# facebookresearch/unbiased-teacher-v2

Measured on AMD Instinct MI355X. Metric: images/sec/node (labeled+unlabeled) UTv2 step, R50-FPN 1333x800, higher is better.
Workload: dtype f16

## Files before the change

include/utv2.h:

```cpp
#ifndef UTV2_H
#define UTV2_H
#include <stdint.h>
#ifdef __cplusplus
extern "C" {
#endif

typedef struct ihipStream_t* utv2_stream_t;

int utv2_conv2d_nhwc_fwd(const float* x, const float* w, float* y, const float* scale, const float* bias,
                         const float* residual, int N, int H, int W, int C, int K, int KH, int KW, int stride, int pad,
                         int in_dil, int OH, int OW, int relu, int accumulate, int Kred, utv2_stream_t stream);
int utv2_conv2d_stem_fwd(const float* x, const float* w, void* y, int y_dtype, const float* scale, const float* bias, int N,
                         int H, int W, int K, int KH, int KW, int stride, int pad, int OH, int OW, int relu, int Kred,
                         utv2_stream_t stream);
int utv2_conv2d_wgrad_splits(int N, int OH, int OW, int K, int Kred);
int64_t utv2_conv2d_wgrad_workspace_floats(int N, int OH, int OW, int K, int Kred);
int utv2_conv2d_nhwc_wgrad(const float* x, const float* dy, float* dw, float* ws, int N, int H, int W, int C, int K,
                           int KH, int KW, int stride, int pad, int OH, int OW, int accumulate, utv2_stream_t stream);
int utv2_colsum(const float* g, float* db, float* ws, int M, int C, int accumulate, utv2_stream_t stream);
int utv2_weight_flip_transpose(const float* w, float* wt, int K, int KH, int KW, int C, utv2_stream_t stream);

int utv2_conv2d_ml_fwd(const float* x, const float* w, float* y, const float* scale, const float* bias,
                       const float* residual, int nlev, const int* H_host, const int* W_host, int N, int C, int K, int KH,
                       int KW, int pad, int relu, int accumulate, utv2_stream_t stream);
// ... 9 lines not shown
int utv2_conv2d_nhwc_fwd_bf16_bits(const void* x, int x_dtype, const void* w16, void* y, int y_dtype, const float* scale,
                                   const float* bias, const void* residual, const void* mask, const void* post_mask, int N, int H, int W,
                                   int C, int K, int KH, int KW, int stride, int pad, int in_dil, int OH, int OW, int relu, int accumulate,
                                   const int* rowinfo, void* relu_bits, const void* mask_bits, const void* post_mask_bits,
                                   utv2_stream_t stream);
int utv2_conv2d_ml_fwd_bf16_g(const void* x, int x_dtype, int x_pitch, const void* w16, void* y, int y_dtype, int y_pitch,
                              const float* scale, const float* bias, const void* residual, int nlev, const int* H_host,
                              const int* W_host, int N, int C, int K, int KH, int KW, int pad, int relu, int accumulate, int groups,
                              float* gn_part, const int* rowinfo, utv2_stream_t stream);
int utv2_conv2d_ml_fwd_bf16_gnb(const void* x, int x_pitch, const void* w16, void* y, int nlev, const int* H_host, const int* W_host, int N,
                                int C, int K, int KH, int KW, int pad, int groups, const int* rowinfo, const void* mask_bits,
                                const void* gnb_x, float* gnb_part, utv2_stream_t stream);
int utv2_conv2d_wgrad_bf16_splits(int M, int K, int Kred);
int64_t utv2_conv2d_wgrad_bf16_workspace_floats(int M, int K, int Kred);
int utv2_conv2d_wgrad_bf16_g(const void* x, int x_dtype, int x_pitch, const void* dy, int dy_dtype, int dy_pitch, float* dw, float* db,
                             float* ws, const int* rowinfo, const float* rowscale, int M, int C, int K, int KH, int KW, int accumulate,
                             int groups, utv2_stream_t stream);
int utv2_conv2d_wgrad_bf16_d(const void* x, int x_dtype, int x_pitch, const void* dy, int dy_dtype, int dy_pitch, float* dw, float* db,
                             float* ws, const int* rowinfo, const float* rowscale, int M, int C, int K, int KH, int KW, int accumulate,
                             int groups, void* pending, utv2_stream_t stream);
int64_t utv2_wgrad_fold_table_bytes(void);
int utv2_wgrad_fold_pending(const void* pending);
int utv2_wgrad_fold_flush(void* pending, utv2_stream_t stream);
int utv2_conv2d_stem_fwd_bf16(const void* xpad16, const void* w16s, void* y, int y_dtype, const float* scale,
                              const float* bias, int N, int H, int W, int K, int OH, int OW, int relu, utv2_stream_t stream);
int utv2_rowinfo_nhwc(int* out, int N, int H, int W, int OH, int OW, int stride, int pad, int KH, int KW, int64_t start,
                      utv2_stream_t stream);
int utv2_f32_to_bf16(const float* src, void* dst16, int64_t n, utv2_stream_t stream);
int utv2_weight_flip_transpose_bf16(const float* w, void* wt16, const float* scale, int K, int KH, int KW, int C,
                                    utv2_stream_t stream);
int utv2_pad_cols_bf16(const void* src, int src_dtype, void* dst16, int64_t rows, int c, int cpad, utv2_stream_t stream);
int utv2_weight_flip_transpose_bf16_batched(const float* arena, const float* scales, void* bank, const void* table, int nlayers,
                                            utv2_stream_t stream);

int utv2_ema_axpby(float* teacher, const float* student, int64_t n, double keep_rate, utv2_stream_t stream);
int utv2_sgd_momentum(float* param, float* grad, float* mom_buf, int64_t n, float lr, float momentum, float weight_decay,
                      float grad_scale, int zero_grad, utv2_stream_t stream);
int utv2_amp_found_inf(const float* grad, int64_t n, float* state, utv2_stream_t stream);
int utv2_sgd_momentum_amp(float* param, const float* grad, float* mom_buf, int64_t n, float lr, float momentum, float weight_decay,
                          float grad_scale, const float* state, utv2_stream_t stream);
int utv2_amp_update_scale(float* state, float growth_factor, float backoff_factor, int growth_interval, utv2_stream_t stream);
int utv2_ema_axpby_m16(float* teacher, const float* student, void* mirror16, int64_t n, double keep_rate, utv2_stream_t stream);
int utv2_sgd_momentum_m16(float* param, float* grad, float* mom_buf, void* mirror16, int64_t n, float lr, float momentum, float weight_decay,
                          float grad_scale, int zero_grad, utv2_stream_t stream);
int utv2_sgd_momentum_amp_m16(float* param, const float* grad, float* mom_buf, void* mirror16, int64_t n, float lr, float momentum,
                              float weight_decay, float grad_scale, const float* state, utv2_stream_t stream);
// ... 242 lines not shown
```

unbiased-teacher-v2_amd/csrc/conv_bf16.hip:

```cpp
#include <mutex>
#include <stdlib.h>
#include "common.h"
#include <type_traits>

__device__ uint4 g_zero64[4] = {{0, 0, 0, 0}, {0, 0, 0, 0}, {0, 0, 0, 0}, {0, 0, 0, 0}};

#define CONV_MAX_LEVELS 8
struct LevelTab {
  int n;
  int start[CONV_MAX_LEVELS + 1];
  int H[CONV_MAX_LEVELS], W[CONV_MAX_LEVELS];
};

struct ConvArgs16 {
  LevelTab lt;
  const void* x;
  const h16_t* w;
  void* y;
  const float* scale;
  const float* bias;
  const void* residual;
  const void* mask;
  const void* post_mask;
  int N, H, W, C, OH, OW, K, KH, KW, stride, pad, in_dil, relu, Kred, M, accumulate;
// ... 1464 lines not shown

int utv2_weight_flip_transpose_bf16_batched(const float* arena, const float* scales, void* bank, const void* table, int nlayers,
                                            hipStream_t stream) {
  if (!arena || !bank || !table || nlayers < 1) return UTV2_EARG;
  static_assert(sizeof(FlipDesc) == 48, "table record layout is part of the ABI");
  hipLaunchKernelGGL(weight_flip_transpose_bf16_batched_kernel, dim3(512, nlayers), dim3(256), 0, stream, arena, scales, (h16_t*)bank,
                     (const FlipDesc*)table);
  return utv2_launch_status();
}

}

struct Wgrad16Args {
  const void* x;
  const void* dy;
  float* ws;
  const int2* rowinfo;
  float* bias_ws;
  int C, K, KH, KW, Kred, M, splits, chunks_per_split;
  int xs;
  int groups;
  int dys;
  int debug;
};

__device__ __forceinline__ bf16x4_t lds_read_tr16(const unsigned char* p) {
  typedef short s16x4 __attribute__((ext_vector_type(4)));
  const s16x4 v = __builtin_amdgcn_ds_read_tr16_b64_v4i16((__attribute__((address_space(3))) s16x4*)p);
  return __builtin_bit_cast(bf16x4_t, v);
}

template <typename TX, typename TDY>
__global__ __launch_bounds__(256) void conv_wgrad_bf16(Wgrad16Args p) {
  constexpr int BK = 32, LDR = 320;
  constexpr int OPB = BK * LDR;
  constexpr bool X16 = sizeof(TX) == 2, DY16 = sizeof(TDY) == 2;
  __shared__ __attribute__((aligned(16))) unsigned char smem[2 * 2 * OPB];
  const int tid = threadIdx.x, lane = tid & 63, wid = tid >> 6;
  const int wm = wid >> 1, wn = wid & 1;
  const int tilesN = (p.Kred + 127) / 128, tilesM = (p.K + 127) / 128;
  const int tiles = tilesM * tilesN;
  int split, bid;
  if ((p.splits & 7) == 0) {
    const int xcd = blockIdx.x & 7, idx = blockIdx.x >> 3;
    split = xcd + 8 * (idx / tiles);
    bid = idx % tiles;
  } else {
    split = blockIdx.x / tiles;
    bid = blockIdx.x - split * tiles;
  }
  const int mt = bid / tilesN, nt = bid - mt * tilesN;
  const int i0 = mt * 128, j0 = nt * 128;
  const int goff = p.groups > 1 ? (i0 / (p.K / p.groups)) * p.C : 0;

  const int cg = tid & 15, pl0 = tid >> 4;
  const int co8 = i0 + cg * 8;
  const bool aok = co8 < p.K;
  const int kk = j0 + cg * 8;
  const bool bok = kk < p.Kred;
  const int tap = bok ? kk / p.C : 0;
  const int ci = bok ? kk - tap * p.C : 0;
  const int dh = tap / p.KW, dw = tap - dh * p.KW;

  f32x16 acc[2][2];
#pragma unroll
  for (int i = 0; i < 2; ++i)
#pragma unroll
    for (int j = 0; j < 2; ++j)
#pragma unroll
      for (int e = 0; e < 16; ++e) acc[i][j][e] = 0.f;

  const int chunk_begin = split * p.chunks_per_split;
  const int total_chunks = (p.M + BK - 1) / BK;
  int chunk_end = chunk_begin + p.chunks_per_split;
  if (chunk_end > total_chunks) chunk_end = total_chunks;

  int2 ri[2];
  bf16x8_t ra[2], rb[2];
  float bsum[8];
#pragma unroll
  for (int e = 0; e < 8; ++e) bsum[e] = 0.f;
  const bool do_bias = p.bias_ws != nullptr && nt == 0;

  auto rload = [&](int chunk) {
#pragma unroll
    for (int r = 0; r < 2; ++r) {
      int m = chunk * BK + pl0 + 16 * r;
      m = m < p.M ? m : p.M - 1;
      ri[r] = p.rowinfo[m];
    }
  };
  auto load8 = [&](const void* base, size_t eoff, bool is16, bool ok) -> bf16x8_t {
    bf16x8_t v;
    if (is16) {
      const h16_t* src = ok ? (const h16_t*)base + eoff : (const h16_t*)g_zero64;
      v = *(const bf16x8_t*)src;
    } else {
      const float* src = ok ? (const float*)base + eoff : (const float*)g_zero64;
      const f32x4 v0 = *(const f32x4*)src, v1 = *(const f32x4*)(src + 4);
#pragma unroll
      for (int e = 0; e < 4; ++e) {
        v[e] = (h16_t)v0[e];
        v[4 + e] = (h16_t)v1[e];
      }
    }
    return v;
  };
  auto load_piece = [&](int chunk, int q) {
    const int r = q & 1;
    const int m = chunk * BK + pl0 + 16 * r;
    const bool mok = m < p.M;
    if (q < 2) {
      ra[r] = load8(p.dy, (size_t)m * p.dys + co8, DY16, mok && aok);
    } else {
      const int W = ri[r].y >> 16;
      const bool ok = mok && bok && ((ri[r].y >> tap) & 1);
      rb[r] = load8(p.x, (size_t)(ri[r].x + dh * W + dw) * p.xs + goff + ci, X16, ok);
    }
  };
  auto store_piece = [&](int buf, int q) {
    const int r = q & 1;
    unsigned char* dst = smem + buf * 2 * OPB + (q < 2 ? 0 : OPB) + (pl0 + 16 * r) * LDR + cg * 16;
    if (q < 2) {
      *(bf16x8_t*)dst = ra[r];
      if (do_bias) {
#pragma unroll
        for (int e = 0; e < 8; ++e) bsum[e] += (float)ra[r][e];
      }
    } else {
      *(bf16x8_t*)dst = rb[r];
    }
  };

  const int G = lane >> 4, t = lane & 15;
// ... 346 lines not shown
  __shared__ float red[256];
  const int c = blockIdx.x * 32 + (threadIdx.x & 31), part = threadIdx.x >> 5;
  float s[4] = {0.f, 0.f, 0.f, 0.f};
  if (c < K) {
    int b = part;
    for (; b + 24 < nb; b += 32) {
#pragma unroll
      for (int u = 0; u < 4; ++u) s[u] += partial[(size_t)(b + 8 * u) * K + c];
    }
    for (; b < nb; b += 8) s[0] += partial[(size_t)b * K + c];
  }
  red[threadIdx.x] = (s[0] + s[1]) + (s[2] + s[3]);
  __syncthreads();
  if (part == 0 && c < K) {
    float v = 0.f;
#pragma unroll
    for (int k = 0; k < 8; ++k) v += red[threadIdx.x + 32 * k];
    if (rowscale) v *= rowscale[c];
    db[c] = accumulate ? db[c] + v : v;
  }
}

__global__ __launch_bounds__(256) void reduce_slabs16_f32(const float* __restrict__ ws, float* __restrict__ dst, size_t n, int splits,
                                                          int accumulate, const float* __restrict__ rowscale, int rowlen) {
  const size_t n4 = n >> 2;
  size_t i = (size_t)blockIdx.x * blockDim.x + threadIdx.x;
  const size_t stride = (size_t)gridDim.x * blockDim.x;
  for (; i < n4; i += stride) {
    f32x4 s[4];
#pragma unroll
    for (int u = 0; u < 4; ++u) s[u] = f32x4{0.f, 0.f, 0.f, 0.f};
    int k = 0;
    for (; k + 4 <= splits; k += 4) {
#pragma unroll
      for (int u = 0; u < 4; ++u) s[u] += ((const f32x4*)(ws + (size_t)(k + u) * n))[i];
    }
    for (; k < splits; ++k) s[0] += ((const f32x4*)(ws + (size_t)k * n))[i];
    f32x4 t = (s[0] + s[1]) + (s[2] + s[3]);
    if (rowscale) {
      const float r = rowscale[(i * 4) / rowlen];
#pragma unroll
      for (int e = 0; e < 4; ++e) t[e] *= r;
    }
    if (accumulate) t += ((const f32x4*)dst)[i];
    ((f32x4*)dst)[i] = t;
  }
}

__global__ void reduce_slabs16_scalar_f32(const float* __restrict__ ws, float* __restrict__ dst, size_t n, int splits, int accumulate,
                                          const float* __restrict__ rowscale) {
  size_t i = (size_t)blockIdx.x * blockDim.x + threadIdx.x;
  if (i >= n) return;
  float s = 0.f;
  for (int k = 0; k < splits; ++k) s += ws[(size_t)k * n + i];
  if (rowscale) s *= rowscale[i];
  dst[i] = accumulate ? dst[i] + s : s;
}

#define SLAB_FOLD_MAX 24
struct SlabFold {
  const float* ws;
  float* dst;
  const float* rowscale;
  unsigned long long n;
  int splits, accumulate, rowlen, kind;
  int blk0, nblk;
};
struct SlabFoldTable {
  int count, total_blocks;
  SlabFold e[SLAB_FOLD_MAX];
};

__global__ __launch_bounds__(256) void reduce_slabs_table(SlabFoldTable t) {
  __shared__ float red[256];
  int ei = 0;
  for (int i = 1; i < t.count; ++i)
    if ((int)blockIdx.x >= t.e[i].blk0) ei = i;
  const SlabFold f = t.e[ei];
  const int lb = (int)blockIdx.x - f.blk0;
  if (f.kind == 0) {
    const size_t n4 = f.n >> 2;
    const size_t stride = (size_t)f.nblk * 256;
    for (size_t i = (size_t)lb * 256 + threadIdx.x; i < n4; i += stride) {
      f32x4 s[4];
#pragma unroll
      for (int u = 0; u < 4; ++u) s[u] = f32x4{0.f, 0.f, 0.f, 0.f};
      int k = 0;
      for (; k + 4 <= f.splits; k += 4) {
#pragma unroll
        for (int u = 0; u < 4; ++u) s[u] += ((const f32x4*)(f.ws + (size_t)(k + u) * f.n))[i];
      }
      for (; k < f.splits; ++k) s[0] += ((const f32x4*)(f.ws + (size_t)k * f.n))[i];
      f32x4 v = (s[0] + s[1]) + (s[2] + s[3]);
      if (f.rowscale) {
        const float r = f.rowscale[(i * 4) / f.rowlen];
#pragma unroll
        for (int e = 0; e < 4; ++e) v[e] *= r;
      }
      if (f.accumulate) v += ((const f32x4*)f.dst)[i];
      ((f32x4*)f.dst)[i] = v;
    }
// ... 8 lines not shown
    const int K = (int)f.n, nb = f.splits;
    const int c = lb * 32 + (threadIdx.x & 31), part = threadIdx.x >> 5;
    float s[4] = {0.f, 0.f, 0.f, 0.f};
    if (c < K) {
      int b = part;
      for (; b + 24 < nb; b += 32) {
#pragma unroll
        for (int u = 0; u < 4; ++u) s[u] += f.ws[(size_t)(b + 8 * u) * K + c];
      }
      for (; b < nb; b += 8) s[0] += f.ws[(size_t)b * K + c];
    }
    red[threadIdx.x] = (s[0] + s[1]) + (s[2] + s[3]);
    __syncthreads();
    if (part == 0 && c < K) {
      float v = 0.f;
#pragma unroll
      for (int k = 0; k < 8; ++k) v += red[threadIdx.x + 32 * k];
      if (f.rowscale) v *= f.rowscale[c];
      f.dst[c] = f.accumulate ? f.dst[c] + v : v;
    }
  }
}

static int slab_fold_add(SlabFoldTable* t, int kind, const float* ws, float* dst, const float* rowscale, size_t n, int splits, int accumulate,
                         int rowlen) {
  if (t->count < 0 || t->count >= SLAB_FOLD_MAX) return UTV2_EARG;
  for (int i = 0; i < t->count; ++i)
    if (t->e[i].dst == dst) return UTV2_EARG;
  SlabFold& f = t->e[t->count];
  f.kind = kind; f.ws = ws; f.dst = dst; f.rowscale = rowscale; f.n = n; f.splits = splits; f.accumulate = accumulate; f.rowlen = rowlen;
  int nb;
  if (kind == 0) { nb = cdiv((int64_t)n / 4, 256); if (nb > 2048) nb = 2048; }
  else if (kind == 1) nb = cdiv((int64_t)n, 256);
  else nb = cdiv((int64_t)n, 32);
  if (nb < 1) nb = 1;
  f.blk0 = t->count == 0 ? 0 : t->e[t->count - 1].blk0 + t->e[t->count - 1].nblk;
  f.nblk = nb;
  t->total_blocks = f.blk0 + nb;
  ++t->count;
  return UTV2_OK;
}

extern "C" {

static int wgrad16_small_splits(int M, int K, int Kred) {
  const int chunks = cdiv(M, 32);
  const int tiles = cdiv(K, 128) * cdiv(Kred, 128);
  const double flop = 2.0 * M * K * Kred;
  int splits = cdiv(flop > 512 * 2.0e8 ? 1024 : 512, tiles);
  const int max_by_chunks = chunks / 8 > 0 ? chunks / 8 : 1;
  if (splits > max_by_chunks) splits = max_by_chunks;
  if (splits < 1) splits = 1;
  if (splits > 256) splits = 256;
// ... 23 lines not shown
    return false;
  if (KH * KW == 1 && chunks < 16 * (256 / tiles)) return false;
  return true;
}

int utv2_conv2d_wgrad_bf16_splits(int M, int K, int Kred) { return wgrad16_small_splits(M, K, Kred); }

int utv2_colsum_partials(const float* partial, float* db, int nb, int K, int accumulate, hipStream_t stream) {
  if (!partial || !db || nb < 1 || K < 1) return UTV2_EARG;
  hipLaunchKernelGGL(colsum_final_f32, dim3(cdiv(K, 32)), dim3(256), 0, stream, partial, db, nb, K, accumulate, (const float*)nullptr);
  return utv2_launch_status();
}

int64_t utv2_conv2d_wgrad_bf16_workspace_floats(int M, int K, int Kred) {
  int64_t n = (int64_t)wgrad16_small_splits(M, K, Kred) * ((int64_t)K * Kred + K);
  if ((K & 255) == 0 && (Kred & 255) == 0) {
    const int64_t n8 = (int64_t)wgrad16_w8_splits(M, K, Kred) * K * Kred + (int64_t)WGRAD_W8_MAX_NB * K;
    if (n8 > n) n = n8;
  }
  return n;
}

static int wgrad16_tail(SlabFoldTable* pending, int kind, const float* src, float* dst, const float* rowscale, size_t n, int parts,
                        int accumulate, int rowlen, hipStream_t stream) {
  if (pending) return slab_fold_add(pending, kind, src, dst, rowscale, n, parts, accumulate, rowlen);
  if (kind == 0) {
    int rb = cdiv((int64_t)n / 4, 256);
    if (rb > 8192) rb = 8192;
    hipLaunchKernelGGL(reduce_slabs16_f32, dim3(rb), dim3(256), 0, stream, src, dst, n, parts, accumulate, rowscale, rowlen);
  } else if (kind == 1) {
    hipLaunchKernelGGL(reduce_slabs16_scalar_f32, dim3(cdiv((int64_t)n, 256)), dim3(256), 0, stream, src, dst, n, parts, accumulate, rowscale);
  } else {
    hipLaunchKernelGGL(colsum_final_f32, dim3(cdiv((int64_t)n, 32)), dim3(256), 0, stream, src, dst, parts, (int)n, accumulate, rowscale);
  }
  return UTV2_OK;
}

static int wgrad_bf16_impl(const void* x, int x_dtype, int x_pitch, const void* dy, int dy_dtype, int dy_pitch, float* dw, float* db,
                           float* ws, const int* rowinfo, const float* rowscale, int M, int C, int K, int KH, int KW, int accumulate,
                           int groups, hipStream_t stream, SlabFoldTable* pending) {
  if (!x || !dy || !dw || !ws || !rowinfo || (C & 7) || (K & 7) || M <= 0 || KH * KW > 16 || bad_dtype(x_dtype) ||
      bad_dtype(dy_dtype) || groups < 1 || K % groups || x_pitch < groups * C || (groups > 1 && (K / groups) % 128) ||
      (x_pitch != C && (x_pitch & (x_dtype == UTV2_BF16 ? 7 : 3))) || dy_pitch < K || (dy_pitch != K && (dy_pitch & (dy_dtype == UTV2_BF16 ? 7 : 3))))
    return UTV2_EARG;
  Wgrad16Args a;
  a.x = x; a.dy = dy; a.ws = ws; a.rowinfo = (const int2*)rowinfo;
  a.C = C; a.K = K; a.KH = KH; a.KW = KW; a.Kred = KH * KW * C; a.M = M; a.debug = 0; a.xs = x_pitch; a.groups = groups; a.dys = dy_pitch;
  const size_t n = (size_t)K * a.Kred;
  if (g_use_wgrad_w8 && x_dtype == UTV2_BF16 && dy_dtype == UTV2_BF16 && dy_pitch == K && wgrad16_w8_shape_ok(M, C, K, KH, KW, x_pitch, groups)) {
    a.splits = wgrad16_w8_splits(M, K, a.Kred);
    a.chunks_per_split = cdiv(cdiv(M, WGRAD_W8_BP), a.splits);
    a.bias_ws = nullptr;
    const int smem = 2 * 2 * WGRAD_W8_BP * 512;
    static LdsOptIn pp_opt_in;
    pp_opt_in({(const void*)conv_wgrad_bf16_pp}, smem);
    hipLaunchKernelGGL(conv_wgrad_bf16_pp, dim3(wgrad16_w8_budget()), dim3(512), smem, stream, a);
    if (int rc = wgrad16_tail(pending, 0, ws, dw, rowscale, n, a.splits, accumulate, a.Kred, stream)) return rc;
    if (db) {
      float* part = ws + (size_t)a.splits * n;
      int nb = cdiv(M, 64);
      if (nb > WGRAD_W8_MAX_NB) nb = WGRAD_W8_MAX_NB;
      const int rows = cdiv(M, nb);
      nb = cdiv(M, rows);
      hipLaunchKernelGGL(colsum_bf16_partial, dim3(nb), dim3(256), 0, stream, (const h16_t*)dy, part, M, K, rows);
      if (int rc = wgrad16_tail(pending, 2, part, db, rowscale, (size_t)K, nb, accumulate, 1, stream)) return rc;
    }
    return utv2_launch_status();
  }
  a.splits = wgrad16_small_splits(M, K, a.Kred);
  a.chunks_per_split = cdiv(cdiv(M, 32), a.splits);
// ... 4 lines not shown
  if (int rc = wgrad16_tail(pending, 0, ws, dw, rowscale, n, a.splits, accumulate, a.Kred, stream)) return rc;
  if (db)
    if (int rc = wgrad16_tail(pending, 1, a.bias_ws, db, rowscale, (size_t)K, a.splits, accumulate, 1, stream)) return rc;
  return utv2_launch_status();
}

int utv2_conv2d_wgrad_bf16_g(const void* x, int x_dtype, int x_pitch, const void* dy, int dy_dtype, int dy_pitch, float* dw, float* db,
                             float* ws, const int* rowinfo, const float* rowscale, int M, int C, int K, int KH, int KW, int accumulate,
                             int groups, hipStream_t stream) {
  return wgrad_bf16_impl(x, x_dtype, x_pitch, dy, dy_dtype, dy_pitch, dw, db, ws, rowinfo, rowscale, M, C, K, KH, KW, accumulate, groups,
                         stream, nullptr);
}

int utv2_conv2d_wgrad_bf16_d(const void* x, int x_dtype, int x_pitch, const void* dy, int dy_dtype, int dy_pitch, float* dw, float* db,
                             float* ws, const int* rowinfo, const float* rowscale, int M, int C, int K, int KH, int KW, int accumulate,
                             int groups, void* pending, hipStream_t stream) {
  if (!pending) return UTV2_EARG;
  SlabFoldTable* t = (SlabFoldTable*)pending;
  if (t->count < 0 || t->count + 3 > SLAB_FOLD_MAX) return UTV2_EARG;
  return wgrad_bf16_impl(x, x_dtype, x_pitch, dy, dy_dtype, dy_pitch, dw, db, ws, rowinfo, rowscale, M, C, K, KH, KW, accumulate, groups,
                         stream, t);
}

int64_t utv2_wgrad_fold_table_bytes(void) { return (int64_t)sizeof(SlabFoldTable); }

int utv2_wgrad_fold_pending(const void* pending) { return pending ? ((const SlabFoldTable*)pending)->count : -1; }

int utv2_wgrad_fold_flush(void* pending, hipStream_t stream) {
  if (!pending) return UTV2_EARG;
  SlabFoldTable* t = (SlabFoldTable*)pending;
  if (t->count < 0 || t->count > SLAB_FOLD_MAX) return UTV2_EARG;
  if (t->count == 0) return UTV2_OK;
  hipLaunchKernelGGL(reduce_slabs_table, dim3(t->total_blocks), dim3(256), 0, stream, *t);
  t->count = 0;
  t->total_blocks = 0;
  return utv2_launch_status();
}

}
```

unbiased-teacher-v2_amd/ubteacher/hip.py:

```python
import ctypes
import os

import torch

_HERE = os.path.dirname(os.path.abspath(__file__))
_LIB_DIR = os.environ.get("UTV2_LIB_DIR") or os.path.join(os.path.dirname(_HERE), "lib")
LIB_PATH = os.path.join(_LIB_DIR, "libutv2_hip.so")
LIB_PATHS = {"bf16": LIB_PATH, "fp16": os.path.join(_LIB_DIR, "libutv2_hip_f16.so")}
H16 = ["bf16"]


_H16_DT = [torch.bfloat16]


def set_h16(kind):
    assert kind in LIB_PATHS
    H16[0] = kind
    _H16_DT[0] = torch.bfloat16 if kind == "bf16" else torch.float16


def h16_dtype():
    return _H16_DT[0]

_lib = None
# ... 18 lines not shown
        for a in [x.strip() for x in args.replace("\n", " ").split(",") if x.strip()]:
            if "*" in a or "utv2_stream_t" in a:
                argt.append(c_p)
            elif a.startswith("int64_t"):
                argt.append(c_i64)
            elif a.startswith("double"):
                argt.append(ctypes.c_double)
            elif a.startswith("float"):
                argt.append(c_f)
            elif a.startswith("int"):
                argt.append(c_i)
            elif a == "void":
                pass
            else:
                raise RuntimeError("utv2.h: cannot map argument %r of %s" % (a, name))
        sigs[name] = (c_i64 if ret == "int64_t" else c_i, argt)
    return sigs


_SIGS = _parse_header(HEADER_PATH)
_PLAIN = {"utv2_aug_resize_workspace_bytes", "utv2_topk_rows_workspace_bytes", "utv2_groupnorm_seg_workspace_floats", "utv2_groupnorm_seg_chunks", "utv2_conv2d_wgrad_bf16_splits", "utv2_conv2d_wgrad_bf16_workspace_floats", "utv2_conv2d_bf16_supported", "utv2_conv2d_wgrad_splits", "utv2_conv2d_wgrad_workspace_floats", "utv2_groupnorm_workspace_floats",
          "utv2_nms_mpad", "utv2_nms_workspace_bytes", "utv2_bottleneck_supported", "utv2_wgrad_fold_table_bytes", "utv2_wgrad_fold_pending",
          "utv2_coco_eval_workspace_bytes", "utv2_gconv3x3_supported", "utv2_gconv3x3_wgrad_splits",
          "utv2_gconv3x3_wgrad_workspace_floats"}


_libs = {}


def load(kind=None):
    kind = kind or H16[0]
    lib = _libs.get(kind)
    if lib is not None:
        return lib
    path = LIB_PATHS[kind]
    if not os.path.exists(path):
        raise RuntimeError(
            "HIP extension %s is missing - run `python __graft_entry__.py` (hipcc, gfx950)" % path
        )
    lib = ctypes.CDLL(path)
    for name, (res, args) in _SIGS.items():
        fn = getattr(lib, name)
        fn.restype = res
        fn.argtypes = args
    _libs[kind] = lib
    return lib

# ... 1137 lines not shown
WGRAD_FOLD = [None]


def conv2d_wgrad_bf16(x, dy2d, dw, rowinfo, C, kh, kw, accumulate=True, db=None, rowscale=None, groups=1, x_pitch=None):
    M, K = dy2d.shape
    assert dy2d.stride(1) == 1
    dy_pitch = int(dy2d.stride(0))
    nws = load().utv2_conv2d_wgrad_bf16_workspace_floats(M, K, kh * kw * C)
    pitch = int(x_pitch) if x_pitch is not None else groups * C
    xp = _p(x) if pitch == C else x.data_ptr()
    dyp = _p(dy2d) if dy_pitch == K else dy2d.data_ptr()
    lane = WGRAD_FOLD[0]
    if lane is not None:
        ws = lane.take(nws, dy2d.device, [dw.data_ptr()] + ([db.data_ptr()] if db is not None else []))
        call("utv2_conv2d_wgrad_bf16_d", xp, _dt(x), pitch, dyp, _dt(dy2d), dy_pitch, _p(dw), _p(db), _p(ws), _p(rowinfo), _p(rowscale), M, C,
             K, kh, kw, int(accumulate), int(groups), ctypes.cast(lane.table, c_p), _stream())
    else:
        ws = workspace(nws, dy2d.device, "wgrad")
        call("utv2_conv2d_wgrad_bf16_g", xp, _dt(x), pitch, dyp, _dt(dy2d), dy_pitch, _p(dw), _p(db), _p(ws), _p(rowinfo), _p(rowscale), M, C,
             K, kh, kw, int(accumulate), int(groups), _stream())
    return dw


def gconv3x3_supported(C, groups):
    return bool(load().utv2_gconv3x3_supported(C, groups))


def _gconv_check(t, w, groups):
    C = t.shape[-1]
    assert t.dim() == 4 and t.dtype == w.dtype and tuple(w.shape) == (C, 9 * C // groups), (tuple(t.shape), tuple(w.shape), groups)
    assert gconv3x3_supported(C, groups), (C, groups)
    return C


def gconv3x3_fwd(x, w, groups, stride=1, scale=None, shift=None, relu=False, out_dtype=None, out=None):
    N, H, W, C = x.shape
    _gconv_check(x, w, groups)
    OH, OW = conv_out_size(H, 3, stride, 1), conv_out_size(W, 3, stride, 1)
    if out is None:
        out = torch.empty((N, OH, OW, C), dtype=out_dtype or x.dtype, device=x.device)
    assert tuple(out.shape) == (N, OH, OW, C)
    call("utv2_gconv3x3_fwd", _p(x), _p(w), _dt(x), _p(out), _dt(out), _p(scale), _p(shift), N, H, W, C, groups, stride, OH, OW,
         int(relu), _stream())
    return out


# ... 215 lines not shown
```

unbiased-teacher-v2_amd/ubteacher/modeling/fcos.py:

```python
import math

import os

import torch

from .. import hip, ops
from ..d2.registry import PROPOSAL_GENERATOR_REGISTRY
from ..d2.structures import Boxes, Instances
from ..utils import comm
from .backbone import _nchw_view

INF = 100000000
METHODS = {"cls": 0, "cls_n_ctr": 1, "ctr": 2, "cls_n_loc": 3}
BOX_STRIDE = 80
BOX_STRIDE_CONT = 16


class PaddedBoxes:

    def __init__(self, image_sizes, **fields):
        self.image_sizes = image_sizes
        self.f = fields

    def __getitem__(self, k):
# ... 281 lines not shown
        def init_box(t):
            t.zero_()
            t[:R4].normal_(0.0, 0.01)
            if has_std:
                t[R4:R4 + 4].normal_(0.0, 0.0001)
            t[R4 + 4:R4 + 5].normal_(0.0, 0.01)

        def rows(r0, r1):
            def fn(t):
                return t[r0:r1].view(r1 - r0, 3, 3, C).permute(0, 3, 1, 2)
            return fn

        wb = store.new((bs, 9 * C), "decay", init_box)
        wb.export(prefix + ".bbox_pred.weight", rows(0, R4))
        if has_std:
            wb.export(prefix + ".bbox_pred_std.weight", rows(R4, R4 + 4))
        wb.export(prefix + ".ctrness.weight", rows(R4 + 4, R4 + 5))
        bb = store.new((bs,), "decay", lambda t: t.zero_())
        bb.export(prefix + ".bbox_pred.bias", lambda t: t[0:R4])
        if has_std:
            bb.export(prefix + ".bbox_pred_std.bias", lambda t: t[R4:R4 + 4])
        bb.export(prefix + ".ctrness.bias", lambda t: t[R4 + 4:R4 + 5])
        self.box_head = ops.Conv(wb, C, bs, 3, 1, 1, bias=bb, colscale=R4, out_fp32=True)
        self.box_head.dgrad_pad_small = not self.reg_discrete
        self.scales = None
        if fc.USE_SCALE:
            self.scales = [store.new((1,), "decay", lambda t: t.fill_(1.0)).export("%s.scales.%d.scale" % (prefix, l))
                           for l in range(self.num_levels)]

    def __call__(self, big, meta):
        t = big
        if self.paired:
            for conv, gn in self.towers["pair"]:
                t = gn(conv(t, meta=meta), meta)
            tc, tb = ops.split_cols(t)
        else:
            for conv, gn in self.towers["share"]:
                t = gn(conv(t, meta=meta), meta)
            tc = t
            for conv, gn in self.towers["cls"]:
                tc = gn(conv(tc, meta=meta), meta)
            tb = t
            for conv, gn in self.towers["bbox"]:
                tb = gn(conv(tb, meta=meta), meta)
        logits = self.cls_logits(tc, meta=meta)
        box = self.box_head(tb, meta=meta, colscale_handle=self.scales)
# ... 387 lines not shown
```

unbiased-teacher-v2_amd/ubteacher/ops.py:

```python
import os

import torch

from . import hip

_HOOKS = {}
PRECISION = ["fp32"]


def set_precision(p):
    assert p in ("fp32", "bf16", "fp16")
    PRECISION[0] = p
    hip.set_h16("fp16" if p == "fp16" else "bf16")


def amp():
    return PRECISION[0] != "fp32"


def act_dtype():
    return hip.h16_dtype() if amp() else torch.float32


_VERSION = [0]
# ... 270 lines not shown
            ent = (cur, img)
            self.single[id(layer)] = ent
        return ent[1]


class Conv:

    def __init__(self, w, cin, cout, k, stride=1, pad=0, bias=None, bn=None, relu=False, trainable=True,
                 kred=None, colscale=None, out_fp32=False, groups=1):
        self.w = w
        self.cin, self.cout, self.k, self.stride, self.pad = cin, cout, k, stride, pad
        self.groups = groups
        self.gconv = groups > 1 and bn is not None
        assert groups == 1 or (colscale is None and cout % groups == 0)
        assert not self.gconv or (k == 3 and pad == 1 and stride in (1, 2) and cin * groups == cout and bias is None
                                  and cin % 4 == 0)
        self.bias = bias
        self.bn = bn
        self.relu = relu
        self.trainable = trainable
        self.kred = kred if kred is not None else k * k * cin
        self.colscale = colscale
        self.out_fp32 = out_fp32
        self.dgrad_pad_small = False
        self.premask_input = False
        self.bias_by_gn = False
        self.gn_cpg = 0
        self._gn_part = None
        self.gnb_src = None
        self.grad_premasked = False
        self._wt = None
        self._wt_version = -1

    def scale_shift(self):
        if self.bn is not None:
            return self.bn.scale, self.bn.shift
        return None, (self.bias.t if self.bias is not None else None)

    def wt(self):
        v = (_VERSION[0], self.w.store.version)
        if self._wt is None or self._wt_version != v:
            self._wt = hip.weight_flip_transpose(self.w.t, self.cout, self.k, self.k, self.cin)
            self._wt_version = v
        return self._wt

    def wt16(self, scale=None):
# ... 178 lines not shown
                    other = ctx.fanin.take() if ctx.fanin is not None else None
                    if other is not None and (other.dtype != x.dtype or tuple(other.shape) != tuple(x.shape)):
                        raise RuntimeError("FanIn: stored gradient does not match the conv input")
                    dest = ctx.pair[0].grad_half(ctx.pair[1], x) if (ctx.pair is not None and other is None) else None
                    wt = layer.wt16(wsc)
                    if (ctx.gnb is not None and other is None and dest is None and x.dtype == hip.h16_dtype()
                            and hip.gnb_eligible(gp, wt, layer.k, layer.k - 1 - layer.pad, G)):
                        src, gx, bits = ctx.gnb
                        part = hip.gnb_part_buffer(x.shape[0], x.shape[1], x.device)
                        dx = hip.conv2d_ml_fwd_bf16(gp, wt, meta.level_hw, meta.N, k=layer.k, pad=layer.k - 1 - layer.pad, out_dtype=x.dtype,
                                                    groups=G, gnb=(bits, gx, part))
                        src._gnb_bwd = (dx.data_ptr(), part)
                    else:
                        dx = hip.conv2d_ml_fwd_bf16(gp, wt, meta.level_hw, meta.N, k=layer.k, pad=layer.k - 1 - layer.pad,
                                                    residual=other, out_dtype=x.dtype, out=dest, groups=G)
                elif G > 1:
                    dx = torch.cat([hip.conv2d_ml_dgrad(g[:, gi * Kg:(gi + 1) * Kg].contiguous(),
                                                        hip.weight_flip_transpose(layer.w.t[gi * Kg:(gi + 1) * Kg], Kg, layer.k, layer.k, layer.cin),
                                                        meta.level_hw, meta.N, layer.k, layer.pad) for gi in range(G)], dim=1)
                else:
                    dx = hip.conv2d_ml_dgrad(g, layer.wt(), meta.level_hw, meta.N, layer.k, layer.pad)
            if layer.use_bf16_wgrad():
                gw = gp[:, :layer.cout] if (d16 and ctx.needs_input_grad[0] and gp is not g) else g
                _wgrad_launch(lambda: hip.conv2d_wgrad_bf16(
                    x, gw, layer.w.g, hip.rowinfo_ml(meta.N, meta.level_hw, layer.pad, layer.k, x.device), layer.cin, layer.k, layer.k,
                    accumulate=True, db=layer.bias.g if (layer.bias is not None and not layer.bias_grad_from_gn()) else None, rowscale=wsc,
                    groups=G, x_pitch=x.stride(0)), x, gw, key=layer)
                bias_done = True
            elif G > 1:
                for gi in range(G):
                    xg, gg = x[:, gi * layer.cin:(gi + 1) * layer.cin].contiguous(), g[:, gi * Kg:(gi + 1) * Kg].contiguous()
                    _wgrad_launch(lambda xg=xg, gg=gg, gi=gi: hip.conv2d_ml_wgrad(xg, gg, layer.w.g[gi * Kg:(gi + 1) * Kg], meta.level_hw, meta.N,
                                                                                   layer.k, layer.pad, accumulate=True), xg, gg, key=layer)
            else:
                _wgrad_launch(lambda: hip.conv2d_ml_wgrad(x, g, layer.w.g, meta.level_hw, meta.N, layer.k, layer.pad, accumulate=True), x, g, key=layer)
        else:
            x4 = x.view(1, x.shape[0], 1, x.shape[1]) if meta is not None else x
            g4 = g.view(1, g.shape[0], 1, g.shape[1]) if meta is not None else g
            if ctx.needs_input_grad[0]:
                pm = x4 if (layer.premask_input and premask_on()) else None
                if d16 and layer.k == 1 and layer.stride == 2 and layer.pad == 0:
                    dxc = hip.conv2d_fwd_bf16(g4, layer.wt16(wsc), out_dtype=x.dtype)
                    dx = hip.zero_interleave2x(dxc, x4.shape[1], x4.shape[2], mask=pm)
                elif (d16 and layer.k == 3 and layer.stride == 2 and layer.pad == 1 and g4.shape[-1] % 32 == 0
                      and x4.shape[0] * x4.shape[1] * x4.shape[2] <= 65536):
                    gd = hip.zero_interleave2x(g4.contiguous(), x4.shape[1], x4.shape[2])
                    dx = hip.conv2d_fwd_bf16(gd, layer.wt16(wsc), pad=1, kh=3, kw=3, out_dtype=x.dtype, mask=pm)
# ... 313 lines not shown


def split_cols(t):
    C = t.shape[1] // 2
    if not (torch.is_grad_enabled() and t.requires_grad):
        return t[:, :C], t[:, C:]
    pair = ColPair()
    a, b = _SplitColsFn.apply(t, pair)
    a._utv2_pair, b._utv2_pair = (pair, 0), (pair, 1)
    return a, b


def pair_conv_gn(conv, gn):
    conv.bias_by_gn = True
    conv.gn_cpg = conv.cout // gn.groups
    gn.bias_conv = conv
    return conv, gn


def gn_bwd_fuse_on():
    return os.environ.get("UTV2_GN_BWD_FUSE", "1") != "0"


def chain_gn_conv(gn, conv):
    gn.next_conv = conv
    conv.gnb_src = gn
    return conv


class GroupNormReLU:
    def __init__(self, gamma, beta, groups=32, eps=1e-5, relu=True):
        self.gamma, self.beta, self.groups, self.eps, self.relu = gamma, beta, groups, eps, relu
        self.bias_conv = None
        self.next_conv = None
        self._gnb_fwd = None
        self._gnb_bwd = None

    def __call__(self, x, meta=None):
        if torch.is_grad_enabled():
            return _GNFn.apply(x, hook(x.device), self, meta)
        return self._fwd(x, meta)[0]

    def _fwd(self, x, meta, for_backward=False):
        if meta is None:
            N, H, W, C = x.shape
            y, mean, rstd = hip.groupnorm_relu_seg_fwd(x.view(-1, C), [H * W] * N, self.gamma.t, self.beta.t, self.groups, self.eps,
# ... 369 lines not shown
```

Before: 354.4.

## Compact nonzero gradient rows for FCOS box-head weight-gradient conv

Adds a two-kernel row-compaction pass that finds rows of the box-head output gradient that are nonzero (only positive locations get regression gradients), gathers them with their rowinfo into a compact buffer capped at about M/8, and runs the bf16 wgrad kernel over only those rows. If the count exceeds the cap, a dense fallback kernel variant runs instead, and the slab reduction selects the split count on device. It aims to skip the GEMM work on zero rows, at the cost of an extra scan and gather over dy and launching both kernel variants, one of which exits early.

```diff
diff --git a/include/utv2.h b/include/utv2.h
--- a/include/utv2.h
+++ b/include/utv2.h
@@ -55,6 +55,15 @@
 int64_t utv2_wgrad_fold_table_bytes(void);
 int utv2_wgrad_fold_pending(const void* pending);
 int utv2_wgrad_fold_flush(void* pending, utv2_stream_t stream);
+int utv2_rows_compact_cap(int M);
+int64_t utv2_rows_compact_workspace_ints(int M);
+int utv2_rows_nonzero_compact(const void* dy16, int dy_pitch, int K, int M, const int* rowinfo, int cap, int* count, int* rows, void* dy_c,
+                              int* rowinfo_c, int* ws, utv2_stream_t stream);
+int64_t utv2_conv2d_wgrad_bf16_sparse_workspace_floats(int M, int cap, int K, int Kred);
+int utv2_conv2d_wgrad_bf16_sparse(const void* x, int x_dtype, int x_pitch, const void* dy, int dy_pitch, const void* dy_c,
+                                  const int* rowinfo_c, const int* count, int cap, float* dw, float* db, float* ws, const int* rowinfo,
+                                  const float* rowscale, int M, int C, int K, int KH, int KW, int accumulate, void* pending,
+                                  utv2_stream_t stream);
 int utv2_conv2d_stem_fwd_bf16(const void* xpad16, const void* w16s, void* y, int y_dtype, const float* scale,
                               const float* bias, int N, int H, int W, int K, int OH, int OW, int relu, utv2_stream_t stream);
 int utv2_rowinfo_nhwc(int* out, int N, int H, int W, int OH, int OW, int stride, int pad, int KH, int KW, int64_t start,
diff --git a/unbiased-teacher-v2_amd/csrc/conv_bf16.hip b/unbiased-teacher-v2_amd/csrc/conv_bf16.hip
--- a/unbiased-teacher-v2_amd/csrc/conv_bf16.hip
+++ b/unbiased-teacher-v2_amd/csrc/conv_bf16.hip
@@ -1510,6 +1510,8 @@
   int groups;
   int dys;
   int debug;
+  const int* count;
+  int cap;
 };
 
 __device__ __forceinline__ bf16x4_t lds_read_tr16(const unsigned char* p) {
@@ -1518,9 +1520,18 @@
   return __builtin_bit_cast(bf16x4_t, v);
 }
 
-template <typename TX, typename TDY>
+template <typename TX, typename TDY, int SP = 0>
 __global__ __launch_bounds__(256) void conv_wgrad_bf16(Wgrad16Args p) {
   constexpr int BK = 32, LDR = 320;
+  int M = p.M, chunks_per_split = p.chunks_per_split;
+  if constexpr (SP != 0) {
+    const int cnt = *p.count;
+    if ((SP == 1) == (cnt > p.cap)) return;
+    if constexpr (SP == 1) {
+      M = cnt;
+      chunks_per_split = ((M + BK - 1) / BK + p.splits - 1) / p.splits;
+    }
+  }
   constexpr int OPB = BK * LDR;
   constexpr bool X16 = sizeof(TX) == 2, DY16 = sizeof(TDY) == 2;
   __shared__ __attribute__((aligned(16))) unsigned char smem[2 * 2 * OPB];
@@ -1558,9 +1569,9 @@
 #pragma unroll
       for (int e = 0; e < 16; ++e) acc[i][j][e] = 0.f;
 
-  const int chunk_begin = split * p.chunks_per_split;
-  const int total_chunks = (p.M + BK - 1) / BK;
-  int chunk_end = chunk_begin + p.chunks_per_split;
+  const int chunk_begin = split * chunks_per_split;
+  const int total_chunks = (M + BK - 1) / BK;
+  int chunk_end = chunk_begin + chunks_per_split;
   if (chunk_end > total_chunks) chunk_end = total_chunks;
 
   int2 ri[2];
@@ -1574,7 +1585,7 @@
 #pragma unroll
     for (int r = 0; r < 2; ++r) {
       int m = chunk * BK + pl0 + 16 * r;
-      m = m < p.M ? m : p.M - 1;
+      m = m < M ? m : M - 1;
       ri[r] = p.rowinfo[m];
     }
   };
@@ -1597,7 +1608,7 @@
   auto load_piece = [&](int chunk, int q) {
     const int r = q & 1;
     const int m = chunk * BK + pl0 + 16 * r;
-    const bool mok = m < p.M;
+    const bool mok = m < M;
     if (q < 2) {
       ra[r] = load8(p.dy, (size_t)m * p.dys + co8, DY16, mok && aok);
     } else {
@@ -1990,7 +2001,9 @@
 }
 
 __global__ __launch_bounds__(256) void reduce_slabs16_f32(const float* __restrict__ ws, float* __restrict__ dst, size_t n, int splits,
-                                                          int accumulate, const float* __restrict__ rowscale, int rowlen) {
+                                                          int accumulate, const float* __restrict__ rowscale, int rowlen,
+                                                          const int* __restrict__ count, int cap, int splits_over) {
+  if (count && *count > cap) splits = splits_over;
   const size_t n4 = n >> 2;
   size_t i = (size_t)blockIdx.x * blockDim.x + threadIdx.x;
   const size_t stride = (size_t)gridDim.x * blockDim.x;
@@ -2016,7 +2029,8 @@
 }
 
 __global__ void reduce_slabs16_scalar_f32(const float* __restrict__ ws, float* __restrict__ dst, size_t n, int splits, int accumulate,
-                                          const float* __restrict__ rowscale) {
+                                          const float* __restrict__ rowscale, const int* __restrict__ count, int cap, int splits_over) {
+  if (count && *count > cap) splits = splits_over;
   size_t i = (size_t)blockIdx.x * blockDim.x + threadIdx.x;
   if (i >= n) return;
   float s = 0.f;
@@ -2033,6 +2047,8 @@
   unsigned long long n;
   int splits, accumulate, rowlen, kind;
   int blk0, nblk;
+  const int* count;
+  int cap, splits_over;
 };
 struct SlabFoldTable {
   int count, total_blocks;
@@ -2044,7 +2060,8 @@
   int ei = 0;
   for (int i = 1; i < t.count; ++i)
     if ((int)blockIdx.x >= t.e[i].blk0) ei = i;
-  const SlabFold f = t.e[ei];
+  SlabFold f = t.e[ei];
+  if (f.count && *f.count > f.cap) f.splits = f.splits_over;
   const int lb = (int)blockIdx.x - f.blk0;
   if (f.kind == 0) {
     const size_t n4 = f.n >> 2;
@@ -2099,13 +2116,19 @@
   }
 }
 
+struct SlabPick {
+  const int* count;
+  int cap, splits_over;
+};
+
 static int slab_fold_add(SlabFoldTable* t, int kind, const float* ws, float* dst, const float* rowscale, size_t n, int splits, int accumulate,
-                         int rowlen) {
+                         int rowlen, SlabPick pick) {
   if (t->count < 0 || t->count >= SLAB_FOLD_MAX) return UTV2_EARG;
   for (int i = 0; i < t->count; ++i)
     if (t->e[i].dst == dst) return UTV2_EARG;
   SlabFold& f = t->e[t->count];
   f.kind = kind; f.ws = ws; f.dst = dst; f.rowscale = rowscale; f.n = n; f.splits = splits; f.accumulate = accumulate; f.rowlen = rowlen;
+  f.count = pick.count; f.cap = pick.cap; f.splits_over = pick.splits_over;
   int nb;
   if (kind == 0) { nb = cdiv((int64_t)n / 4, 256); if (nb > 2048) nb = 2048; }
   else if (kind == 1) nb = cdiv((int64_t)n, 256);
@@ -2175,14 +2198,17 @@
 }
 
 static int wgrad16_tail(SlabFoldTable* pending, int kind, const float* src, float* dst, const float* rowscale, size_t n, int parts,
-                        int accumulate, int rowlen, hipStream_t stream) {
-  if (pending) return slab_fold_add(pending, kind, src, dst, rowscale, n, parts, accumulate, rowlen);
+                        int accumulate, int rowlen, hipStream_t stream, SlabPick pick = SlabPick{nullptr, 0, 0}) {
+  if (pending) return slab_fold_add(pending, kind, src, dst, rowscale, n, parts, accumulate, rowlen, pick);
+  if (pick.count && kind == 2) return UTV2_EARG;
   if (kind == 0) {
     int rb = cdiv((int64_t)n / 4, 256);
     if (rb > 8192) rb = 8192;
-    hipLaunchKernelGGL(reduce_slabs16_f32, dim3(rb), dim3(256), 0, stream, src, dst, n, parts, accumulate, rowscale, rowlen);
+    hipLaunchKernelGGL(reduce_slabs16_f32, dim3(rb), dim3(256), 0, stream, src, dst, n, parts, accumulate, rowscale, rowlen, pick.count,
+                       pick.cap, pick.splits_over);
   } else if (kind == 1) {
-    hipLaunchKernelGGL(reduce_slabs16_scalar_f32, dim3(cdiv((int64_t)n, 256)), dim3(256), 0, stream, src, dst, n, parts, accumulate, rowscale);
+    hipLaunchKernelGGL(reduce_slabs16_scalar_f32, dim3(cdiv((int64_t)n, 256)), dim3(256), 0, stream, src, dst, n, parts, accumulate, rowscale,
+                       pick.count, pick.cap, pick.splits_over);
   } else {
     hipLaunchKernelGGL(colsum_final_f32, dim3(cdiv((int64_t)n, 32)), dim3(256), 0, stream, src, dst, parts, (int)n, accumulate, rowscale);
   }
@@ -2199,6 +2225,7 @@
   Wgrad16Args a;
   a.x = x; a.dy = dy; a.ws = ws; a.rowinfo = (const int2*)rowinfo;
   a.C = C; a.K = K; a.KH = KH; a.KW = KW; a.Kred = KH * KW * C; a.M = M; a.debug = 0; a.xs = x_pitch; a.groups = groups; a.dys = dy_pitch;
+  a.count = nullptr; a.cap = 0;
   const size_t n = (size_t)K * a.Kred;
   if (g_use_wgrad_w8 && x_dtype == UTV2_BF16 && dy_dtype == UTV2_BF16 && dy_pitch == K && wgrad16_w8_shape_ok(M, C, K, KH, KW, x_pitch, groups)) {
     a.splits = wgrad16_w8_splits(M, K, a.Kred);
@@ -2249,6 +2276,139 @@
                          stream, t);
 }
 
+#define COMPACT_ROWS 256
+
+__global__ __launch_bounds__(256) void rows_nonzero_flags(const unsigned short* __restrict__ dy, int pitch, int K, int M,
+                                                          unsigned* __restrict__ masks, int* __restrict__ block_counts) {
+  __shared__ unsigned flag[COMPACT_ROWS];
+  __shared__ unsigned long long ball[4];
+  const int tid = threadIdx.x, r0 = blockIdx.x * COMPACT_ROWS;
+  flag[tid] = 0u;
+  __syncthreads();
+  const int cpr = K >> 3;
+  const int rows = M - r0 < COMPACT_ROWS ? M - r0 : COMPACT_ROWS;
+  for (int i = tid; i < rows * cpr; i += 256) {
+    const int r = i / cpr, c = i - r * cpr;
+    const uint4 v = *(const uint4*)(dy + (size_t)(r0 + r) * pitch + c * 8);
+    if (((v.x | v.y | v.z | v.w) & 0x7fff7fffu) != 0u) atomicOr(&flag[r], 1u);
+  }
+  __syncthreads();
+  const unsigned long long b = __ballot(flag[tid] != 0u);
+  if ((tid & 63) == 0) ball[tid >> 6] = b;
+  __syncthreads();
+  if (tid < 8) masks[(size_t)blockIdx.x * 8 + tid] = (unsigned)(ball[tid >> 1] >> (32 * (tid & 1)));
+  if (tid == 0) block_counts[blockIdx.x] = __popcll(ball[0]) + __popcll(ball[1]) + __popcll(ball[2]) + __popcll(ball[3]);
+}
+
+__global__ __launch_bounds__(256) void rows_nonzero_gather(const unsigned short* __restrict__ dy, int pitch, int M, const int2* __restrict__ rowinfo,
+                                                           const unsigned* __restrict__ masks, const int* __restrict__ block_counts,
+                                                           int cap, int* __restrict__ count, int* __restrict__ rows_out,
+                                                           unsigned short* __restrict__ dy_c, int2* __restrict__ rowinfo_c) {
+  __shared__ int red[2][256];
+  __shared__ int slot[COMPACT_ROWS];
+  const int tid = threadIdx.x, nb = gridDim.x, b = blockIdx.x;
+  int before = 0, total = 0;
+  for (int i = tid; i < nb; i += 256) {
+    const int c = block_counts[i];
+    total += c;
+    if (i < b) before += c;
+  }
+  red[0][tid] = before; red[1][tid] = total;
+  __syncthreads();
+  for (int s = 128; s > 0; s >>= 1) {
+    if (tid < s) { red[0][tid] += red[0][tid + s]; red[1][tid] += red[1][tid + s]; }
+    __syncthreads();
+  }
+  before = red[0][0]; total = red[1][0];
+  if (b == 0 && tid == 0) *count = total;
+  const unsigned mw = masks[(size_t)b * 8 + (tid >> 5)];
+  int pre = __popc(mw & ((1u << (tid & 31)) - 1u));
+  for (int w = 0; w < (tid >> 5); ++w) pre += __popc(masks[(size_t)b * 8 + w]);
+  const bool on = (mw >> (tid & 31)) & 1u;
+  const int dst = before + pre;
+  slot[tid] = (on && dst < cap) ? dst : -1;
+  if (on && dst < cap) {
+    rows_out[dst] = b * COMPACT_ROWS + tid;
+    rowinfo_c[dst] = rowinfo[b * COMPACT_ROWS + tid];
+  }
+  __syncthreads();
+  const int cpr = pitch >> 3;
+  for (int i = tid; i < COMPACT_ROWS * cpr; i += 256) {
+    const int r = i / cpr, c = i - r * cpr;
+    const int d = slot[r];
+    if (d >= 0) *(uint4*)(dy_c + (size_t)d * pitch + c * 8) = *(const uint4*)(dy + (size_t)(b * COMPACT_ROWS + r) * pitch + c * 8);
+  }
+  const int used = total < cap ? total : cap;
+  const int per = (cap - used + nb - 1) / nb;
+  const int t0 = used + b * per;
+  int t1 = t0 + per;
+  if (t1 > cap) t1 = cap;
+  for (int j = t0 + tid; j < t1; j += 256) {
+    rows_out[j] = -1;
+    rowinfo_c[j] = make_int2(0, 0);
+  }
+  for (int i = tid; i < (t1 - t0) * cpr; i += 256) {
+    const int r = i / cpr, c = i - r * cpr;
+    *(uint4*)(dy_c + (size_t)(t0 + r) * pitch + c * 8) = make_uint4(0u, 0u, 0u, 0u);
+  }
+}
+
+static int rows_compact_cap(int M) { return ((M + 7) / 8 + 31) / 32 * 32; }
+
+int utv2_rows_compact_cap(int M) { return M > 0 ? rows_compact_cap(M) : 0; }
+
+int64_t utv2_rows_compact_workspace_ints(int M) { return M > 0 ? 9 * (int64_t)cdiv(M, COMPACT_ROWS) : 0; }
+
+int utv2_rows_nonzero_compact(const void* dy16, int dy_pitch, int K, int M, const int* rowinfo, int cap, int* count, int* rows, void* dy_c,
+                              int* rowinfo_c, int* ws, hipStream_t stream) {
+  if (!dy16 || !rowinfo || !count || !rows || !dy_c || !rowinfo_c || !ws || M < 1 || K < 8 || (K & 7) || dy_pitch < K || (dy_pitch & 7) ||
+      cap < 1 || (int64_t)M * dy_pitch >= (1ll << 31))
+    return UTV2_EARG;
+  const int nb = cdiv(M, COMPACT_ROWS);
+  unsigned* masks = (unsigned*)ws;
+  int* block_counts = ws + 8 * (size_t)nb;
+  hipLaunchKernelGGL(rows_nonzero_flags, dim3(nb), dim3(256), 0, stream, (const unsigned short*)dy16, dy_pitch, K, M, masks, block_counts);
+  hipLaunchKernelGGL(rows_nonzero_gather, dim3(nb), dim3(256), 0, stream, (const unsigned short*)dy16, dy_pitch, M, (const int2*)rowinfo,
+                     masks, block_counts, cap, count, rows, (unsigned short*)dy_c, (int2*)rowinfo_c);
+  return utv2_launch_status();
+}
+
+static int wgrad16_sparse_slabs(int M, int cap, int K, int Kred) {
+  const int a = wgrad16_small_splits(cap, K, Kred), b = wgrad16_small_splits(M, K, Kred);
+  return a > b ? a : b;
+}
+
+int64_t utv2_conv2d_wgrad_bf16_sparse_workspace_floats(int M, int cap, int K, int Kred) {
+  return (int64_t)wgrad16_sparse_slabs(M, cap, K, Kred) * ((int64_t)K * Kred + K);
+}
+
+int utv2_conv2d_wgrad_bf16_sparse(const void* x, int x_dtype, int x_pitch, const void* dy, int dy_pitch, const void* dy_c, const int* rowinfo_c,
+                                  const int* count, int cap, float* dw, float* db, float* ws, const int* rowinfo, const float* rowscale, int M,
+                                  int C, int K, int KH, int KW, int accumulate, void* pending, hipStream_t stream) {
+  if (!x || !dy || !dy_c || !rowinfo_c || !count || !dw || !ws || !rowinfo || (C & 7) || (K & 7) || M <= 0 || cap < 32 || (cap & 31) ||
+      cap > M + 31 || KH * KW > 16 || bad_dtype(x_dtype) || x_pitch < C || (x_pitch != C && (x_pitch & (x_dtype == UTV2_BF16 ? 7 : 3))) ||
+      dy_pitch < K || (dy_pitch & 7))
+    return UTV2_EARG;
+  SlabFoldTable* t = (SlabFoldTable*)pending;
+  if (t && (t->count < 0 || t->count + 3 > SLAB_FOLD_MAX)) return UTV2_EARG;
+  Wgrad16Args a;
+  a.x = x; a.ws = ws; a.C = C; a.K = K; a.KH = KH; a.KW = KW; a.Kred = KH * KW * C; a.debug = 0; a.xs = x_pitch; a.groups = 1; a.dys = dy_pitch;
+  a.count = count; a.cap = cap;
+  const size_t n = (size_t)K * a.Kred;
+  const int tiles = cdiv(K, 128) * cdiv(a.Kred, 128);
+  const int splits_s = wgrad16_small_splits(cap, K, a.Kred), splits_d = wgrad16_small_splits(M, K, a.Kred);
+  a.bias_ws = db ? ws + (size_t)wgrad16_sparse_slabs(M, cap, K, a.Kred) * n : nullptr;
+  a.dy = dy_c; a.rowinfo = (const int2*)rowinfo_c; a.M = cap; a.splits = splits_s; a.chunks_per_split = cdiv(cdiv(cap, 32), splits_s);
+  with_type(x_dtype, [&](auto tx) { hipLaunchKernelGGL((conv_wgrad_bf16<TAG_T(tx), h16_t, 1>), dim3(tiles * splits_s), dim3(256), 0, stream, a); });
+  a.dy = dy; a.rowinfo = (const int2*)rowinfo; a.M = M; a.splits = splits_d; a.chunks_per_split = cdiv(cdiv(M, 32), splits_d);
+  with_type(x_dtype, [&](auto tx) { hipLaunchKernelGGL((conv_wgrad_bf16<TAG_T(tx), h16_t, 2>), dim3(tiles * splits_d), dim3(256), 0, stream, a); });
+  const SlabPick pick{count, cap, splits_d};
+  if (int rc = wgrad16_tail(t, 0, ws, dw, rowscale, n, splits_s, accumulate, a.Kred, stream, pick)) return rc;
+  if (db)
+    if (int rc = wgrad16_tail(t, 1, a.bias_ws, db, rowscale, (size_t)K, splits_s, accumulate, 1, stream, pick)) return rc;
+  return utv2_launch_status();
+}
+
 int64_t utv2_wgrad_fold_table_bytes(void) { return (int64_t)sizeof(SlabFoldTable); }
 
 int utv2_wgrad_fold_pending(const void* pending) { return pending ? ((const SlabFoldTable*)pending)->count : -1; }
diff --git a/unbiased-teacher-v2_amd/ubteacher/hip.py b/unbiased-teacher-v2_amd/ubteacher/hip.py
--- a/unbiased-teacher-v2_amd/ubteacher/hip.py
+++ b/unbiased-teacher-v2_amd/ubteacher/hip.py
@@ -64,7 +64,8 @@
 _PLAIN = {"utv2_aug_resize_workspace_bytes", "utv2_topk_rows_workspace_bytes", "utv2_groupnorm_seg_workspace_floats", "utv2_groupnorm_seg_chunks", "utv2_conv2d_wgrad_bf16_splits", "utv2_conv2d_wgrad_bf16_workspace_floats", "utv2_conv2d_bf16_supported", "utv2_conv2d_wgrad_splits", "utv2_conv2d_wgrad_workspace_floats", "utv2_groupnorm_workspace_floats",
           "utv2_nms_mpad", "utv2_nms_workspace_bytes", "utv2_bottleneck_supported", "utv2_wgrad_fold_table_bytes", "utv2_wgrad_fold_pending",
           "utv2_coco_eval_workspace_bytes", "utv2_gconv3x3_supported", "utv2_gconv3x3_wgrad_splits",
-          "utv2_gconv3x3_wgrad_workspace_floats"}
+          "utv2_gconv3x3_wgrad_workspace_floats", "utv2_rows_compact_cap", "utv2_rows_compact_workspace_ints",
+          "utv2_conv2d_wgrad_bf16_sparse_workspace_floats"}
 
 
 _libs = {}
@@ -1248,6 +1249,53 @@
     return dw
 
 
+def rows_compact_cap(M):
+    return int(load().utv2_rows_compact_cap(int(M)))
+
+
+def _ibuf(nints, device, tag):
+    return workspace(nints, device, tag).view(torch.int32)
+
+
+def rows_nonzero_compact(dy2d, rowinfo, out=None):
+    M, K = dy2d.shape
+    assert dy2d.dtype == h16_dtype() and dy2d.stride(1) == 1 and tuple(rowinfo.shape) == (M, 2) and rowinfo.dtype == torch.int32
+    pitch = int(dy2d.stride(0))
+    cap = rows_compact_cap(M)
+    dev = dy2d.device
+    if out is None:
+        meta = _ibuf(3 * cap + 64, dev, "rows_compact")
+        count, rows, ri_c = meta[:1], meta[64:64 + cap], meta[64 + cap:64 + 3 * cap].view(cap, 2)
+        dy_c = workspace((cap * pitch + 1) // 2, dev, "rows_compact_dy").view(h16_dtype())[:cap * pitch].view(cap, pitch)
+    else:
+        count, rows, dy_c, ri_c = out
+        assert tuple(dy_c.shape) == (cap, pitch) and dy_c.dtype == dy2d.dtype and rows.numel() == cap and tuple(ri_c.shape) == (cap, 2)
+    ws = _ibuf(load().utv2_rows_compact_workspace_ints(M), dev, "rows_compact_ws")
+    call("utv2_rows_nonzero_compact", dy2d.data_ptr(), pitch, K, M, _p(rowinfo), cap, _p(count), _p(rows), _p(dy_c), _p(ri_c), _p(ws), _stream())
+    return count, rows, dy_c, ri_c
+
+
+def conv2d_wgrad_bf16_sparse(x, dy2d, dw, rowinfo, C, kh, kw, accumulate=True, db=None, rowscale=None, groups=1, x_pitch=None, compact=None):
+    M, K = dy2d.shape
+    assert groups == 1
+    count, _rows, dy_c, ri_c = compact if compact is not None else rows_nonzero_compact(dy2d, rowinfo)
+    cap = dy_c.shape[0]
+    dy_pitch = int(dy2d.stride(0))
+    nws = load().utv2_conv2d_wgrad_bf16_sparse_workspace_floats(M, cap, K, kh * kw * C)
+    pitch = int(x_pitch) if x_pitch is not None else C
+    xp = _p(x) if pitch == C else x.data_ptr()
+    lane = WGRAD_FOLD[0]
+    if lane is not None:
+        ws = lane.take(nws, dy2d.device, [dw.data_ptr()] + ([db.data_ptr()] if db is not None else []))
+        table = ctypes.cast(lane.table, c_p)
+    else:
+        ws = workspace(nws, dy2d.device, "wgrad")
+        table = None
+    call("utv2_conv2d_wgrad_bf16_sparse", xp, _dt(x), pitch, dy2d.data_ptr(), dy_pitch, _p(dy_c), _p(ri_c), _p(count), cap, _p(dw), _p(db), _p(ws),
+         _p(rowinfo), _p(rowscale), M, C, K, kh, kw, int(accumulate), table, _stream())
+    return dw
+
+
 def gconv3x3_supported(C, groups):
     return bool(load().utv2_gconv3x3_supported(C, groups))
 
diff --git a/unbiased-teacher-v2_amd/ubteacher/modeling/fcos.py b/unbiased-teacher-v2_amd/ubteacher/modeling/fcos.py
--- a/unbiased-teacher-v2_amd/ubteacher/modeling/fcos.py
+++ b/unbiased-teacher-v2_amd/ubteacher/modeling/fcos.py
@@ -327,6 +327,7 @@
             bb.export(prefix + ".bbox_pred_std.bias", lambda t: t[R4:R4 + 4])
         bb.export(prefix + ".ctrness.bias", lambda t: t[R4 + 4:R4 + 5])
         self.box_head = ops.Conv(wb, C, bs, 3, 1, 1, bias=bb, colscale=R4, out_fp32=True)
+        self.box_head.sparse_grad_rows = True
         self.box_head.dgrad_pad_small = not self.reg_discrete
         self.scales = None
         if fc.USE_SCALE:
diff --git a/unbiased-teacher-v2_amd/ubteacher/ops.py b/unbiased-teacher-v2_amd/ubteacher/ops.py
--- a/unbiased-teacher-v2_amd/ubteacher/ops.py
+++ b/unbiased-teacher-v2_amd/ubteacher/ops.py
@@ -316,6 +316,7 @@
         self.kred = kred if kred is not None else k * k * cin
         self.colscale = colscale
         self.out_fp32 = out_fp32
+        self.sparse_grad_rows = False
         self.dgrad_pad_small = False
         self.premask_input = False
         self.bias_by_gn = False
@@ -540,7 +541,9 @@
                     dx = hip.conv2d_ml_dgrad(g, layer.wt(), meta.level_hw, meta.N, layer.k, layer.pad)
             if layer.use_bf16_wgrad():
                 gw = gp[:, :layer.cout] if (d16 and ctx.needs_input_grad[0] and gp is not g) else g
-                _wgrad_launch(lambda: hip.conv2d_wgrad_bf16(
+                sparse = layer.sparse_grad_rows and G == 1 and gw.dtype == hip.h16_dtype() and gw.stride(0) % 8 == 0 and sparse_head_bwd_on()
+                wgrad = hip.conv2d_wgrad_bf16_sparse if sparse else hip.conv2d_wgrad_bf16
+                _wgrad_launch(lambda: wgrad(
                     x, gw, layer.w.g, hip.rowinfo_ml(meta.N, meta.level_hw, layer.pad, layer.k, x.device), layer.cin, layer.k, layer.k,
                     accumulate=True, db=layer.bias.g if (layer.bias is not None and not layer.bias_grad_from_gn()) else None, rowscale=wsc,
                     groups=G, x_pitch=x.stride(0)), x, gw, key=layer)
@@ -900,6 +903,10 @@
     return os.environ.get("UTV2_GN_BWD_FUSE", "1") != "0"
 
 
+def sparse_head_bwd_on():
+    return os.environ.get("UTV2_SPARSE_HEAD_BWD", "1") != "0"
+
+
 def chain_gn_conv(gn, conv):
     gn.next_conv = conv
     conv.gnb_src = gn
```

After: 357.0, median of 6. No clear change (+0.7%).
